# guzba/zippy

Measured on NVIDIA H100. Metric: compress_level1_gzip_input_throughput, higher is better.
Workload: dtype u8

## Files before the change

zippy_b200/csrc/zb_deflate.cu:

```cuda
#include "zb_device.cuh"
#include "zb_kernels.h"

#define LZ_THREADS (ZB_WARPS_PER_CHUNK * 32)
#define LZ_HASH_BITS 11
#define LZ_TABLE_ENTRIES (1 << LZ_HASH_BITS)
#define LZ_PRESEED 2048
#ifndef ZB_LZ1_RESOLVE_WINNER
#define ZB_LZ1_RESOLVE_WINNER 0
#endif
#define LZ_LANE_CAP 32

#define LZ_PIECE_BYTES ZB_REC_PIECE_BYTES
#define LZ_PHASES (ZB_SUB_BYTES / LZ_PIECE_BYTES)
#define LZ_PHASE_BYTES (ZB_CHUNK_BYTES / LZ_PHASES)
#define LZ_PHASE_HIST 1024
#define LZ_BATCH_LPW 2
#define LZ_BATCH_WINDOWS (32 / LZ_BATCH_LPW)
static_assert(LZ_PIECE_BYTES * ZB_WARPS_PER_CHUNK == LZ_PHASE_BYTES, "one piece per warp and phase");
static_assert(LZ_PIECE_BYTES / ZB_WINDOW % LZ_BATCH_WINDOWS == 0, "a batch of windows never straddles two pieces");

#define LZ_SM_DATA 0
#define LZ_SM_DATA_BYTES (LZ_PHASE_BYTES + LZ_PHASE_HIST + 64 + 384)
#define LZ_SM_TABLE (LZ_SM_DATA + LZ_SM_DATA_BYTES)
#define LZ_SM_TABLE_BYTES (ZB_WARPS_PER_CHUNK * LZ_TABLE_ENTRIES * 2)
#define LZ_SM_HIST (LZ_SM_TABLE + LZ_SM_TABLE_BYTES)
#define LZ_SM_HIST_BYTES (ZB_WARPS_PER_CHUNK * ZB_HIST_WORDS * 4)
#define LZ_SM_RING (LZ_SM_HIST + LZ_SM_HIST_BYTES)
#define LZ_SM_RING_BYTES (ZB_WARPS_PER_CHUNK * LZ_BATCH_WINDOWS * ZB_MATCH_SLOTS * 4)
#define LZ_SM_LMUL (LZ_SM_RING + LZ_SM_RING_BYTES)
#define LZ_LMUL_PIECE 33
#define LZ_LMUL_PQ 49
#define LZ_SM_LMUL_BYTES (56 * 4)
#define LZ_SM_PART (LZ_SM_LMUL + LZ_SM_LMUL_BYTES)
#define LZ_SM_PART_BYTES (ZB_WARPS_PER_CHUNK * 24)
#define LZ_SM_BAR (LZ_SM_PART + LZ_SM_PART_BYTES)
#define LZ_SM_TOTAL (LZ_SM_BAR + 16)
static_assert(LZ_TABLE_ENTRIES * 2 >= 4096, "a warp's table region must hold the CRC step table");
static_assert(3 * (LZ_SM_TOTAL + 1024) <= 233472, "three CTAs per SM");
static_assert(LZ_SM_PART % 8 == 0 && LZ_SM_TABLE % 16 == 0, "alignment");

__device__ __forceinline__ uint32_t lz_hash(uint32_t v) { return (v * 0x9E3779B1u) >> (32 - LZ_HASH_BITS); }
__device__ __forceinline__ uint32_t shl_clamp(uint32_t x, uint32_t n) {
  uint32_t r;
  asm("shl.b32 %0, %1, %2;" : "=r"(r) : "r"(x), "r"(n));
  return r;
}
__device__ __forceinline__ uint32_t low_mask(uint32_t n) { return shl_clamp(1u, n) - 1u; }

__device__ __forceinline__ uint32_t lz_final_rec(uint32_t mlen, uint32_t dist, int &lc, int &dc) {
  uint32_t le, de;
  lc = (int)zb_len_code_bf(mlen, le);
  dc = (int)zb_dist_code_bf(dist, de);
  return (uint32_t)lc | (le << 5) | ((uint32_t)dc << 10) | (de << 15);
}


__device__ __forceinline__ void lz_select(const uint8_t *data, uint32_t off0, uint32_t wb, uint32_t b1, uint32_t cur,
                                          uint32_t nvalid, uint32_t &m, uint32_t dist, uint32_t *ring_slot,
                                          uint32_t &sel, uint32_t &ism, uint32_t &endw) {
  const int lane = zb_lane();
  const uint32_t mm = __ballot_sync(ZB_FULL, m != 0);
  endw = 0;
  ism = 0;
  if (mm) {
    const uint32_t lbit = 1u << lane;
    const uint32_t endp = (uint32_t)lane + m;
    const uint32_t rest = shl_clamp(1u, endp) ? (mm >> endp) : 0u;
    uint32_t nc = rest ? endp + (uint32_t)(__ffs((int)rest) - 1) : 32u;
    uint32_t vis = 1u << (cur + (uint32_t)(__ffs((int)(mm >> cur)) - 1));
#pragma unroll
    for (int r = 0; r < 3; r++) {
      vis |= __reduce_or_sync(ZB_FULL, (vis & lbit) ? shl_clamp(1u, nc) : 0u);
      const uint32_t t = __shfl_sync(ZB_FULL, nc, (int)(nc & 31u));
      nc = nc < 32u ? t : 32u;
    }
    ism = vis;
    const int lastm = 31 - __clz((int)ism);
    const uint32_t cov = (ism & lbit) ? (low_mask(endp) & ~low_mask((uint32_t)lane)) : 0u;
    const uint32_t covered = __reduce_or_sync(ZB_FULL, cov);
    uint32_t mlast = __shfl_sync(ZB_FULL, m, lastm);
    if (mlast >= LZ_LANE_CAP) {
      const uint32_t md = __shfl_sync(ZB_FULL, dist, lastm);
      const uint32_t pos = wb + (uint32_t)lastm;
      const uint32_t off = off0 + pos + LZ_LANE_CAP + 8u * (uint32_t)lane;
      uint32_t x0 = zb_ld32_unaligned(data, off) ^ zb_ld32_unaligned(data, off - md);
      uint32_t x1 = zb_ld32_unaligned(data, off + 4) ^ zb_ld32_unaligned(data, off + 4 - md);
      uint32_t nm = x0 ? ((uint32_t)(__ffs((int)x0) - 1) >> 3) : 4u + (x1 ? ((uint32_t)(__ffs((int)x1) - 1) >> 3) : 4u);
      uint32_t stop = __ballot_sync(ZB_FULL, nm < 8u);
      if (stop) {
        int first = __ffs((int)stop) - 1;
        mlast = LZ_LANE_CAP + 8u * (uint32_t)first + __shfl_sync(ZB_FULL, nm, first);
      } else {
        mlast = LZ_LANE_CAP + 256u;
      }
      mlast = min(mlast, min((uint32_t)ZB_MAX_MATCH, b1 - pos));
      if (lane == lastm) m = mlast;
    }
    sel = ism | (~covered & ~low_mask(cur) & low_mask(nvalid));
    endw = (uint32_t)lastm + mlast;
    if (ism & lbit) {
      uint32_t rank = (uint32_t)__popc(ism & (lbit - 1u));
      ring_slot[rank] = (m - 3u) | ((dist - 1u) << 9);
    }
  } else {
    sel = low_mask(nvalid) & ~low_mask(cur);
  }
}

template <int LPW, bool LITS>
__device__ __forceinline__ void lz_batch_pass(const uint8_t *wdata, bool active, uint32_t ksel, uint32_t kism,
                                              const uint32_t *ring_win, uint32_t *whist, uint2 *gmask_w,
                                              uint32_t *grecs_piece, uint32_t &rec_base) {
  constexpr int NW = 32 / LPW;
  const uint32_t part = (uint32_t)zb_lane() / NW, wi = (uint32_t)zb_lane() % NW;
  if (active && part == 0) *gmask_w = make_uint2(ksel, kism);
  const uint32_t im = active ? kism : 0u;
  const uint32_t pm = (0xffffffffu >> (32 - 32 / LPW)) << (part * (32 / LPW));
  uint32_t s = (LITS && active) ? (ksel & ~kism & pm) : 0u;
  while (s) {
    const uint32_t bit = (uint32_t)(__ffs((int)s) - 1);
    s &= s - 1;
    const uint32_t sy = wdata[bit];
    atomicAdd(&whist[sy >> 1], 1u << ((sy & 1u) * 16u));
  }
  const uint32_t nmatch = (uint32_t)__popc(im);
  uint32_t incl = nmatch;
#pragma unroll
  for (int o = 1; o < NW; o <<= 1) {
    const uint32_t t = __shfl_up_sync(ZB_FULL, incl, o, NW);
    if (wi >= (uint32_t)o) incl += t;
  }
  uint32_t *grecs_w = grecs_piece + rec_base + incl - nmatch;
  rec_base += __shfl_sync(ZB_FULL, incl, NW - 1);
  for (uint32_t k = part; k < nmatch; k += LPW) {
    const uint32_t raw = ring_win[k];
    int lc, dc;
    const uint32_t fin = lz_final_rec((raw & 511u) + 3u, (raw >> 9) + 1u, lc, dc);
    grecs_w[k] = fin;
    const uint32_t s1 = 257u + (uint32_t)lc, s2 = (uint32_t)ZB_NUM_LITLEN + (uint32_t)dc;
    atomicAdd(&whist[s1 >> 1], 1u << ((s1 & 1u) * 16u));
    atomicAdd(&whist[s2 >> 1], 1u << ((s2 & 1u) * 16u));
  }
}

#ifndef ZB_LZ1_STAGE_CLOCKS
#define ZB_LZ1_STAGE_CLOCKS 0
#endif
enum { LZS_WAIT, LZS_CHECKSUM, LZS_SEED, LZS_PROBE, LZS_EXTEND, LZS_SELECT, LZS_BATCH, LZS_BARRIER, LZS_N };
#if ZB_LZ1_STAGE_CLOCKS
__device__ unsigned long long zb_lz1_stage_clk[LZS_N];
#define LZ_CLK_DECL                          \
  unsigned long long clk_acc[LZS_N] = {};    \
  long long clk_t = clock64();
#define LZ_CLK(s)                            \
// ... 397 lines not shown
    lz2_clear_table(own);
    __syncthreads();
    if (rlen) {
      zb_mbar_wait(bar, phase);
      phase ^= 1u;
    }

    const uint32_t b0 = (uint32_t)warp * ZB_SUB_BYTES;
    const uint32_t b1 = min(b0 + ZB_SUB_BYTES, len);
    {
      ZbCheck c;
      c.crc_raw = 0;
      c.a_sum = c.b_sum = 0;
      uint32_t n = b0 < len ? b1 - b0 : 0;
      if (n) {
        c = zb_warp_checksums(data, off0 + b0, n, crc_tab, lane_mul);
        const uint32_t after = len - b1;
        if (after) {
          const uint32_t shift = ((after & (ZB_SUB_BYTES - 1)) == 0) ? lane_mul[33 + after / ZB_SUB_BYTES] : zb_xpow8_t(tabs->pow2, after);
          c.crc_raw = zb_gf2_mul(c.crc_raw, shift);
          c.b_sum += (uint64_t)after * c.a_sum;
        }
      }
      if (lane == 0) {
        part[warp * 3 + 0] = c.crc_raw;
        part[warp * 3 + 1] = c.a_sum;
        part[warp * 3 + 2] = c.b_sum;
      }
      __syncwarp();
    }

    {
      const uint32_t nseg = (hg + rlen + LZ2_SEG_BYTES - 1) / LZ2_SEG_BYTES;
      for (uint32_t sg = (uint32_t)warp; sg + 1 < nseg; sg += ZB_WARPS_PER_CHUNK) {
        uint2 *tab = stat + (size_t)sg * LZ2_BUCKETS;
        lz2_clear_table(tab, (1 << LZ2_STATIC_BITS) * 2);
        __syncwarp();
        uint16_t *tab16 = reinterpret_cast<uint16_t *>(tab);
        const uint32_t q0 = sg ? sg * LZ2_SEG_BYTES - hg : 0u, q1 = (sg + 1) * LZ2_SEG_BYTES - hg;
        for (uint32_t s = q0; s < q1; s += 32) {
          const uint32_t q = s + (uint32_t)lane;
          const uint32_t v = zb_ld32_unaligned(data, mis + q);
          const uint32_t hs = lz2_hash_mul(v) >> (32 - LZ2_STATIC_BITS);
          const bool can = q + 4 <= rlen && q < q1;
          const uint32_t grp = __match_any_sync(ZB_FULL, can ? hs : (0x80000000u | (uint32_t)lane));
          if (can && lane == 31 - __clz((int)grp)) __stcg(&tab16[hs], (uint16_t)q);
        }
        __syncwarp();
      }
    }
    __syncthreads();

    if (b0 < len) {
      const uint32_t myseg = (hg + hb + b0) / LZ2_SEG_BYTES;
      uint32_t entry = b0;
      uint32_t ksel = 0, kism = 0;
      uint2 *gmask = masks + (size_t)chunk * ZB_WINDOWS_PER_CHUNK;
      uint32_t *grecs = recs + (size_t)chunk * ZB_RECS_PER_CHUNK;
      uint32_t rec_base = 0;
      for (uint32_t wb = b0; wb < b1; wb += 32) {
        const uint32_t win = wb >> 5, slot = win & (LZ2_RING_WINDOWS - 1u);
        if ((wb & (ZB_REC_PIECE_BYTES - 1u)) == 0u) rec_base = 0;
        const uint32_t p = wb + (uint32_t)lane;
        const uint32_t q = hb + p;
        const uint32_t v = zb_ld32_unaligned(data, off0 + p);
        const bool can = (p + 4 <= len);
        const uint32_t h = lz2_hash(v);
        const uint32_t limit = p < b1 ? min((uint32_t)ZB_MAX_MATCH, b1 - p) : 0u;
        const bool search = entry < wb + 32 && can && p >= entry && limit >= ZB_MIN_MATCH;
        const uint32_t hs = lz2_hash_mul(v) >> (32 - LZ2_STATIC_BITS);
        uint32_t hcand[4];
#pragma unroll
        for (int j = 0; j < 4; j++) {
          hcand[j] = 0xffffu;
          if (search && myseg > (uint32_t)j && prm.hist_segs > (uint32_t)j)
            hcand[j] = __ldcg(reinterpret_cast<const uint16_t *>(stat + (size_t)(myseg - 1u - (uint32_t)j) * LZ2_BUCKETS) + hs);
        }
        uint32_t grp;
        const uint2 bucket = lz2_probe_insert(own, h, can, q - (uint32_t)lane, grp);
        uint32_t sel = 0, ism = 0;
        if (entry < wb + 32) {
          const uint32_t nvalid = min(32u, b1 - wb);
          const uint32_t cur = entry - wb;
          uint32_t m = 0, dist = 1;
          int budget = search ? (int)prm.maxcand : 0;
          Lz2Pos P;
          P.data32 = reinterpret_cast<const uint32_t *>(data);
          P.poff = off0 + p;
          P.q = q;
          P.v = v;
          P.lim = min(q, (uint32_t)ZB_MAX_DIST);
          P.limit = limit;
          P.stop = min(limit, (uint32_t)LZ_LANE_CAP);
          uint32_t nl = 0;
          {
            const uint32_t lower = grp & ((1u << lane) - 1u);
            lz2_verify(P, q - ((uint32_t)lane - (uint32_t)(31 - __clz((int)(lower | 1u)))), search && lower != 0u, dlist, nl);
            lz2_verify(P, bucket.x & 0xffffu, search, dlist, nl);
            if (prm.own_ways > 1) lz2_verify(P, bucket.x >> 16, search, dlist, nl);
            if (prm.own_ways > 2) lz2_verify(P, bucket.y & 0xffffu, search, dlist, nl);
            if (prm.own_ways > 3) lz2_verify(P, bucket.y >> 16, search, dlist, nl);
#pragma unroll
            for (int j = 0; j < 4; j++)
              if (prm.hist_segs > (uint32_t)j) lz2_verify(P, hcand[j], search, dlist, nl);
          }
          const uint32_t rounds = __reduce_max_sync(ZB_FULL, nl);
          for (uint32_t k = 0; k < rounds; k++) {
            if (k < nl && budget > 0 && m < P.stop) lz2_extend(P, data, dlist[k * (uint32_t)LZ_THREADS], prm.good, m, dist, budget);
          }
          const uint32_t mnext = __shfl_down_sync(ZB_FULL, m, 1);
          if (lane < 31 && m != 0 && m < prm.lazy && mnext > m) m = 0;
          uint32_t endw;
          lz_select(data, off0, wb, b1, cur, nvalid, m, dist, ring + slot * ZB_MATCH_SLOTS, sel, ism, endw);
          entry = wb + max(endw, nvalid);
        }
        const uint32_t bl = (uint32_t)lane & (LZ2_RING_WINDOWS - 1u);
        if (bl == slot) {
          ksel = sel;
          kism = ism;
        }
        if (slot == LZ2_RING_WINDOWS - 1u || wb + 32 >= b1) {
          __syncwarp();
          const uint32_t bwin = win - slot + bl;
          lz_batch_pass<32 / LZ2_RING_WINDOWS, true>(data + off0 + (bwin << 5), bl <= slot, ksel, kism, ring + bl * ZB_MATCH_SLOTS,
                                               whist, gmask + bwin,
                                               grecs + ((wb & ~(uint32_t)(ZB_REC_PIECE_BYTES - 1u)) >> 2), rec_base);
          ksel = kism = 0;
          __syncwarp();
        }
      }
    }
    __syncthreads();
    {
      uint32_t *gh = reinterpret_cast<uint32_t *>(hist + (size_t)chunk * ZB_WARPS_PER_CHUNK * ZB_HIST_SYMS);
      for (int i = tid; i < ZB_WARPS_PER_CHUNK * ZB_HIST_WORDS; i += LZ_THREADS) gh[i] = hist_all[i];
    }
    if (tid == 0) {
      uint32_t raw = 0;
      uint64_t a = 0, b = 0;
      for (int w = 0; w < ZB_WARPS_PER_CHUNK; w++) {
        raw ^= (uint32_t)part[w * 3 + 0];
        a += part[w * 3 + 1];
        b += part[w * 3 + 2];
      }
      ZbChunkCheck cc;
      cc.crc_raw = raw;
      cc.adler = zb_adler_from_sums(a % ZB_ADLER_MOD, b % ZB_ADLER_MOD, len);
      chk[chunk] = cc;
    }
    __syncthreads();
  }
}

__global__ void __launch_bounds__(64)
    k_huff(const ZbChunkDesc *__restrict__ desc, const uint16_t *__restrict__ hist, ZbCodebook *__restrict__ cb,
           uint32_t n_chunks, int level) {
  uint32_t c = blockIdx.x * blockDim.x + threadIdx.x;
  if (c >= n_chunks) return;
  ZbChunkDesc d = desc[c];
  zb_build_codebook(hist + (size_t)c * ZB_WARPS_PER_CHUNK * ZB_HIST_SYMS, d.len, (d.flags & ZB_CHUNK_LAST) ? 1 : 0,
                    level == 0 ? 0 : -1, &cb[c]);
}

__device__ __forceinline__ uint32_t frame_head_bytes(int fmt, const uint8_t *fname_len, uint32_t m) {
  if (fmt == ZB_DF_GZIP) return 10u + (fname_len ? (uint32_t)fname_len[m] : 0u) + 1u;
  if (fmt == ZB_DF_ZLIB) return 2u;
  return 0u;
}
__device__ __forceinline__ uint32_t frame_tail_bytes(int fmt) {
  return fmt == ZB_DF_GZIP ? 8u : fmt == ZB_DF_ZLIB ? 4u : 0u;
}

#define SCAN_THREADS 1024
__global__ void __launch_bounds__(SCAN_THREADS)
    k_scan(ZbCompressWork w) {
  __shared__ uint64_t warp_tot[32];
  __shared__ uint64_t carry_s;
  const int tid = (int)threadIdx.x, lane = tid & 31, warp = tid >> 5;
  if (tid == 0) carry_s = w.out_base_ptr ? *w.out_base_ptr : w.out_base;
  __syncthreads();
  for (uint32_t base = 0; base < w.n_chunks; base += SCAN_THREADS) {
    uint32_t c = base + (uint32_t)tid;
    uint64_t sz = 0;
    uint32_t head = 0, flags = 0, member = 0;
    if (c < w.n_chunks) {
      ZbChunkDesc d = w.desc[c];
      flags = d.flags;
      member = d.member;
      sz = w.cb[c].total_bytes;
      if (flags & ZB_CHUNK_HEAD) {
        head = frame_head_bytes(w.data_format, w.fname_len, member);
        sz += head;
      }
      if (flags & ZB_CHUNK_LAST) sz += frame_tail_bytes(w.data_format);
    }
    uint64_t incl = sz;
#pragma unroll
    for (int o = 1; o < 32; o <<= 1) {
      uint64_t t = __shfl_up_sync(ZB_FULL, incl, o);
      if (lane >= o) incl += t;
    }
    if (lane == 31) warp_tot[warp] = incl;
    __syncthreads();
    if (warp == 0) {
      uint64_t t = warp_tot[lane], it = t;
#pragma unroll
      for (int o = 1; o < 32; o <<= 1) {
        uint64_t u = __shfl_up_sync(ZB_FULL, it, o);
        if (lane >= o) it += u;
      }
      warp_tot[lane] = it - t;
    }
    __syncthreads();
    uint64_t carry = carry_s;
    uint64_t excl = carry + warp_tot[warp] + incl - sz;
    if (c < w.n_chunks) {
      w.chunk_off[c] = excl + head;
      if (flags & ZB_CHUNK_FIRST) w.member_off[member] = excl;
    }
    __syncthreads();
    if (tid == SCAN_THREADS - 1) carry_s = excl + sz;
    __syncthreads();
  }
  if (tid == 0) w.member_off[w.n_members] = carry_s;
}

__global__ void __launch_bounds__(128)
    k_member_check(ZbCompressWork w) {
  const uint32_t m = (blockIdx.x * blockDim.x + threadIdx.x) >> 5, lane = threadIdx.x & 31u;
  if (m >= w.n_members) return;
  const uint32_t c0 = w.member_first[m], c1 = w.member_first[m + 1];
  const uint32_t per = (c1 - c0 + 31u) / 32u;
  const uint32_t a = min(c1, c0 + lane * per), b = min(c1, a + per);
  uint32_t raw = 0, ad = 1;
  uint64_t bytes = 0;
  for (uint32_t c = a; c < b; c++) {
    const uint32_t l = w.desc[c].len;
    const ZbChunkCheck cc = w.chk[c];
    if (w.data_format == ZB_DF_ZLIB) ad = zb_adler32_combine(ad, cc.adler, l);
    else if (w.data_format == ZB_DF_GZIP)
      raw = zb_gf2_mul(raw, l == ZB_CHUNK_BYTES ? w.tabs->sub_mul[0] : zb_xpow8_t(w.tabs->pow2, l)) ^ cc.crc_raw;
    bytes += l;
  }
  if (c1 - c0 > 1u) {
    for (int o = 1; o < 32; o <<= 1) {
      const uint32_t r_raw = __shfl_down_sync(0xffffffffu, raw, o), r_ad = __shfl_down_sync(0xffffffffu, ad, o);
      const uint64_t r_bytes = __shfl_down_sync(0xffffffffu, bytes, o);
      if ((lane & (uint32_t)(2 * o - 1)) == 0u && r_bytes) {
        if (w.data_format == ZB_DF_ZLIB) ad = zb_adler32_combine(ad, r_ad, r_bytes);
        else if (w.data_format == ZB_DF_GZIP) raw = zb_gf2_mul(raw, zb_xpow8_t(w.tabs->pow2, r_bytes)) ^ r_raw;
        bytes += r_bytes;
      }
    }
  }
  if (lane == 0) {
    if (w.carry_in) {
      const ZbMemberCarry ci = w.carry_in[m];
      if (w.data_format == ZB_DF_ZLIB) ad = zb_adler32_combine(ci.adler, ad, bytes);
      else if (w.data_format == ZB_DF_GZIP) raw = zb_gf2_mul(ci.crc_raw, zb_xpow8_t(w.tabs->pow2, bytes)) ^ raw;
      bytes += ci.bytes;
    }
    if (w.carry_out) {
      ZbMemberCarry co;
      co.crc_raw = raw;
      co.adler = ad;
      co.bytes = bytes;
      w.carry_out[m] = co;
    }
    uint32_t v = 0;
    if (w.data_format == ZB_DF_ZLIB) v = ad;
    else if (w.data_format == ZB_DF_GZIP)
      v = ~(zb_gf2_mul(bytes == ZB_CHUNK_BYTES ? w.tabs->sub_mul[0] : zb_xpow8_t(w.tabs->pow2, bytes), 0xffffffffu) ^ raw);
    w.member_check[m] = v;
    w.member_isize[m] = (uint32_t)bytes;
  }
}

#define PK_ROW_WORDS 17
#define PK_STG_WORDS (PK_ROW_WORDS * 32 + 4)
#define PK_EDGES 10
#define PK_LIT_OFF 1
#define PK_SLOT_WORDS 9
#define PK_REC_OFF (PK_LIT_OFF + 32 * PK_SLOT_WORDS)
static_assert(PK_REC_OFF + 32 * ZB_MATCH_SLOTS + 1 <= PK_STG_WORDS, "a batch's staged inputs fit in stg");
#define PK_CODE_NONE 320

struct PkEdges {
  uint32_t word[PK_EDGES];
  uint32_t val[PK_EDGES];
  uint32_t used[PK_EDGES];
};
__device__ __forceinline__ void pk_edge_or(PkEdges *ed, uint32_t relword, uint32_t bits) {
  int k = 0;
#pragma unroll
  for (int i = PK_EDGES - 1; i >= 0; i--)
    if (ed->word[i] == relword) k = i;
  atomicOr(&ed->val[k], bits);
  ed->used[k] = 1u;
}

__device__ __forceinline__ void pk_append(uint32_t *stg, const uint32_t *rows, uint32_t mybits, uint32_t &bitcur,
                                          uint32_t &sw0, uint32_t piece_start, uint32_t *dstw_rel, PkEdges *ed) {
  const int lane = zb_lane();
  uint32_t incl = mybits;
#pragma unroll
  for (int o = 1; o < 32; o <<= 1) {
    const uint32_t t = __shfl_up_sync(ZB_FULL, incl, o);
    if (lane >= o) incl += t;
  }
  const uint32_t total = __shfl_sync(ZB_FULL, incl, 31);
  uint32_t pos = bitcur + incl - mybits - sw0 * 32u;
  for (uint32_t k = 0; k * 32u < mybits; k++) {
    const uint32_t nb = min(32u, mybits - k * 32u);
    uint32_t v = rows[k * 32 + lane];
    if (nb < 32u) v &= (1u << nb) - 1u;
// ... 138 lines not shown
      uint32_t rec_base = 0;
      for (uint32_t wbase = 0; wbase < nwin; wbase += 32) {
        if (wbase && (wbase & (ZB_REC_PIECE_WINDOWS - 1u)) == 0u) {
          grecs += ZB_REC_PIECE_BYTES / 4;
          rec_base = 0;
        }
        const uint32_t widx = wbase + (uint32_t)lane;
        const uint32_t win = (b0 >> 5) + widx;
        uint2 mk = make_uint2(0u, 0u);
        if (widx < nwin) mk = gmask[win];
        uint32_t s = mk.x;
        const uint32_t im = mk.y;
        const uint32_t nmatch = (uint32_t)__popc(im);
        uint32_t rincl = nmatch;
#pragma unroll
        for (int o = 1; o < 32; o <<= 1) {
          const uint32_t t = __shfl_up_sync(ZB_FULL, rincl, o);
          if (lane >= o) rincl += t;
        }
        const uint32_t rtot = __shfl_sync(ZB_FULL, rincl, 31);
        {
          const uint32_t bbase = b0 + (wbase << 5);
          const uint32_t *pw = reinterpret_cast<const uint32_t *>(src + bbase - mis);
          const uint32_t nword = min(1024u, b1 - bbase) + mis;
#pragma unroll 1
          for (uint32_t k = (uint32_t)lane; 4u * k < nword; k += 32) {
            const uint32_t v = __ldg(pw + k);
            uint32_t *q = stg + PK_LIT_OFF + k + (k >> 3);
            if (k < 256u) *q = v;
            if (k && (k & 7u) == 0u) q[-1] = v;
          }
          const uint32_t *brec = grecs + rec_base;
#pragma unroll 1
          for (uint32_t k = (uint32_t)lane; k < rtot; k += 32) stg[PK_REC_OFF + k] = brec[k];
        }
        rec_base += rtot;
        __syncwarp();
        const uint8_t *lit = reinterpret_cast<const uint8_t *>(stg + PK_LIT_OFF + lane * PK_SLOT_WORDS) + mis;
        uint32_t ri = PK_REC_OFF + rincl - nmatch;
        uint32_t wi = (uint32_t)lane, acc = 0, accn = 0;
        while (s) {
          const uint32_t t1 = s & (0u - s);
          s ^= t1;
          const uint32_t t2 = s & (0u - s);
          const uint32_t l1 = lit[31 - __clz(t1)], l2 = lit[31 - __clz(t2)];
          const uint32_t r = stg[ri];
          const bool is_m = (im & t1) != 0u;
          const bool pair = t2 != 0u && (im & (t1 | t2)) == 0u;
          s ^= pair ? t2 : 0u;
          ri += is_m ? 1u : 0u;
          const uint32_t rec = is_m ? r : 0u;
          const uint32_t sym1 = is_m ? 257u + (rec & 31u) : l1;
          const uint32_t sym2 = is_m ? 288u + ((rec >> 10) & 31u) : pair ? l2 : PK_CODE_NONE;
          const uint32_t e1 = codes[sym1], e2 = codes[sym2];
          pk_put(rows, (e1 & 0xffffu) | ((rec >> 5) & 31u) << __byte_perm(e1, 0u, 0x4442), e1 >> 24, acc, accn, wi);
          pk_put(rows, (e2 & 0xffffu) | (rec >> 15) << __byte_perm(e2, 0u, 0x4442), e2 >> 24, acc, accn, wi);
        }
        rows[wi] = acc;
        __syncwarp();
        for (uint32_t k = (uint32_t)lane; k < PK_REC_OFF - PK_LIT_OFF + rtot; k += 32) stg[PK_LIT_OFF + k] = 0u;
        __syncwarp();
        pk_append(stg, rows, wi - (uint32_t)lane + accn, bitcur, sw0, piece_start, dstw_rel, &ed);
      }
    }
    if (lane == 0 && (bitcur & 31u)) pk_edge_or(&ed, sw0, stg[0]);
  }
  if (tid == 96) {
    const uint32_t e = codes[256];
    uint32_t pos = B0 + cb->eob_bit_start;
    unsigned long long tv = (unsigned long long)(e & 0xffffu);
    uint32_t nb = e >> 24;
    if (!cb->is_final) {
      nb += 3u;
      nb += (8u - ((pos + nb) & 7u)) & 7u;
      tv |= 0xffff0000ull << nb;
      nb += 32u;
    } else {
      nb += (8u - ((pos + nb) & 7u)) & 7u;
    }
    while (nb) {
      const uint32_t rel = pos >> 5, sh = pos & 31u, take = min(nb, 32u - sh);
      const uint32_t bits = (uint32_t)(tv & ((1ull << take) - 1ull)) << sh;
      if (sh == 0 && take == 32u) dstw_rel[rel] = bits;
      else pk_edge_or(&ed, rel, bits);
      tv >>= take;
      pos += take;
      nb -= take;
    }
  }
  __syncthreads();
  if (tid < PK_EDGES && ed.used[tid] && (tid == 0 || ed.word[tid] != ed.word[tid - 1])) {
    const uint32_t rel = ed.word[tid], val = ed.val[tid];
    const uint32_t lo = rel * 32u, hi = lo + 32u;
    if (lo >= B0 && hi <= end_bit) dstw_rel[rel] = val;
    else {
      uint8_t *bp = reinterpret_cast<uint8_t *>(dstw_rel + rel);
      for (uint32_t j = 0; j < 4; j++)
        if (lo + 8u * j >= B0 && lo + 8u * j + 8u <= end_bit) bp[j] = (uint8_t)(val >> (8u * j));
    }
  }
}

static bool zb_is_lz_level(int level) { return level == -1 || level >= 2; }
ZbLz2Params zb_lz2_params(int level) {
  static const ZbLz2Params table[10] = {{4, 4, 4, 8, 16}, {4, 4, 4, 8, 16}, {2, 4, 2, 4, 0},  {2, 4, 3, 4, 6},   {3, 4, 3, 4, 8},
                                        {3, 4, 4, 8, 16}, {4, 4, 4, 8, 16}, {4, 4, 6, 8, 32}, {4, 4, 8, 16, 32}, {4, 4, 8, 32, 64}};
  return table[(level >= 2 && level <= 9) ? level : 6];
}
size_t zb_lz2_table_bytes(int *grid_out) {
  int grid = LZ2_CTAS_PER_SM * zb_sm_count();
  if (grid_out) *grid_out = grid;
  return (size_t)grid * LZ2_TABLES_PER_CTA * LZ2_BUCKETS * sizeof(uint2);
}
typedef void (*ZbLzKernel)(const uint8_t *, const ZbChunkDesc *, uint2 *, uint32_t *, uint16_t *, ZbChunkCheck *,
                           const ZbCrcTables *);
static ZbLzKernel zb_lz_kernel(int mode, int data_format) {
  const int ck = data_format == ZB_DF_GZIP ? ZB_CK_CRC : data_format == ZB_DF_ZLIB ? ZB_CK_ADLER : 0;
  if (mode) return ck == ZB_CK_CRC ? k_lz<1, ZB_CK_CRC> : ck == ZB_CK_ADLER ? k_lz<1, ZB_CK_ADLER> : k_lz<1, 0>;
  return ck == ZB_CK_CRC ? k_lz<0, ZB_CK_CRC> : ck == ZB_CK_ADLER ? k_lz<0, ZB_CK_ADLER> : k_lz<0, 0>;
}
cudaError_t zb_setup_deflate_attrs() {
  cudaError_t e = cudaSuccess;
  static const int fmts[3] = {ZB_DF_GZIP, ZB_DF_ZLIB, ZB_DF_DEFLATE};
  for (int mode = 0; mode < 2; mode++)
    for (int f = 0; f < 3; f++) {
      const ZbLzKernel k = zb_lz_kernel(mode, fmts[f]);
      if (e == cudaSuccess) e = cudaFuncSetAttribute(k, cudaFuncAttributeMaxDynamicSharedMemorySize, LZ_SM_TOTAL);
      if (e == cudaSuccess) e = cudaFuncSetAttribute(k, cudaFuncAttributePreferredSharedMemoryCarveout, cudaSharedmemCarveoutMaxShared);
    }
  if (e == cudaSuccess) e = cudaFuncSetAttribute(k_lz2, cudaFuncAttributeMaxDynamicSharedMemorySize, LZ2_SM_TOTAL);
  cudaFuncAttributes fa;
  if (e == cudaSuccess) e = cudaFuncGetAttributes(&fa, k_huff);
  if (e == cudaSuccess) e = cudaFuncGetAttributes(&fa, k_scan);
  if (e == cudaSuccess) e = cudaFuncGetAttributes(&fa, k_member_check);
  if (e == cudaSuccess) e = cudaFuncGetAttributes(&fa, k_pack);
  return e;
}
cudaError_t zb_launch_lz(const ZbCompressWork &w, cudaStream_t s) {
  if (w.n_chunks == 0) return cudaSuccess;
  if (zb_is_lz_level(w.level)) {
    int grid = 0;
    (void)zb_lz2_table_bytes(&grid);
    if ((uint32_t)grid > w.n_chunks) grid = (int)w.n_chunks;
    k_lz2<<<grid, LZ_THREADS, LZ2_SM_TOTAL, s>>>(w.src, w.desc, w.masks, w.recs, w.hist, w.chk, w.tabs, w.lz2_tables,
                                                 w.n_chunks, zb_lz2_params(w.level));
  } else {
    const ZbLzKernel k = zb_lz_kernel((w.level == -2 || w.level == 0) ? 0 : 1, w.data_format);
    k<<<w.n_chunks, LZ_THREADS, LZ_SM_TOTAL, s>>>(w.src, w.desc, w.masks, w.recs, w.hist, w.chk, w.tabs);
  }
  return cudaGetLastError();
}
cudaError_t zb_launch_huff(const ZbCompressWork &w, cudaStream_t s) {
  if (w.n_chunks == 0) return cudaSuccess;
  k_huff<<<(w.n_chunks + 63) / 64, 64, 0, s>>>(w.desc, w.hist, w.cb, w.n_chunks, w.level);
  return cudaGetLastError();
}
cudaError_t zb_launch_scan(const ZbCompressWork &w, cudaStream_t s) {
  k_scan<<<1, SCAN_THREADS, 0, s>>>(w);
  if (w.n_members) k_member_check<<<(w.n_members + 3) / 4, 128, 0, s>>>(w);
  return cudaGetLastError();
}
cudaError_t zb_launch_pack(const ZbCompressWork &w, cudaStream_t s) {
  if (w.n_chunks == 0) return cudaSuccess;
  k_pack<<<w.n_chunks, LZ_THREADS, 0, s>>>(w);
  return cudaGetLastError();
}
```

Measured before the change: 74.42.

## Build Huffman codebooks with one warp per chunk instead of one thread

Replaces the per-thread codebook builder with a warp-cooperative version. Histogram summing, the rank-based sort, length assignment, canonical code generation, header bit packing and per-warp bit offsets are all spread across lanes and use shared memory per warp. This targets the serial per-thread Huffman construction, which left the huff kernel with few active threads and long latency. The tree build and RLE stay on a single lane, and the added shared-memory footprint and warp synchronisation cost something in return. Optional stage clock instrumentation is compiled out by default.

After: 77.09 (median of 6 runs). +3.6%, better.

```diff
diff --git a/zippy_b200/csrc/zb_deflate.cu b/zippy_b200/csrc/zb_deflate.cu
--- a/zippy_b200/csrc/zb_deflate.cu
+++ b/zippy_b200/csrc/zb_deflate.cu
@@ -1,5 +1,6 @@
 #include "zb_device.cuh"
 #include "zb_kernels.h"
+#include "zb_huff_warp.cuh"
 
 #define LZ_THREADS (ZB_WARPS_PER_CHUNK * 32)
 #define LZ_HASH_BITS 11
@@ -703,15 +704,13 @@
   }
 }
 
-__global__ void __launch_bounds__(64)
-    k_huff(const ZbChunkDesc *__restrict__ desc, const uint16_t *__restrict__ hist, ZbCodebook *__restrict__ cb,
-           uint32_t n_chunks, int level) {
-  uint32_t c = blockIdx.x * blockDim.x + threadIdx.x;
-  if (c >= n_chunks) return;
-  ZbChunkDesc d = desc[c];
-  zb_build_codebook(hist + (size_t)c * ZB_WARPS_PER_CHUNK * ZB_HIST_SYMS, d.len, (d.flags & ZB_CHUNK_LAST) ? 1 : 0,
-                    level == 0 ? 0 : -1, &cb[c]);
-}
+#if ZB_HUFF_STAGE_CLOCKS
+extern "C" int zb200_huff_stage_clocks(unsigned long long *out) {
+  unsigned long long zero[HWS_N] = {};
+  if (cudaMemcpyFromSymbol(out, zb_huff_stage_clk, sizeof(zero)) != cudaSuccess) return -1;
+  return cudaMemcpyToSymbol(zb_huff_stage_clk, zero, sizeof(zero)) == cudaSuccess ? 0 : -1;
+}
+#endif
 
 __device__ __forceinline__ uint32_t frame_head_bytes(int fmt, const uint8_t *fname_len, uint32_t m) {
   if (fmt == ZB_DF_GZIP) return 10u + (fname_len ? (uint32_t)fname_len[m] : 0u) + 1u;
@@ -1156,7 +1155,7 @@
 }
 cudaError_t zb_launch_huff(const ZbCompressWork &w, cudaStream_t s) {
   if (w.n_chunks == 0) return cudaSuccess;
-  k_huff<<<(w.n_chunks + 63) / 64, 64, 0, s>>>(w.desc, w.hist, w.cb, w.n_chunks, w.level);
+  k_huff<<<(w.n_chunks + HW_WARPS - 1) / HW_WARPS, HW_WARPS * 32, 0, s>>>(w.desc, w.hist, w.cb, w.n_chunks, w.level);
   return cudaGetLastError();
 }
 cudaError_t zb_launch_scan(const ZbCompressWork &w, cudaStream_t s) {
diff --git a/zippy_b200/csrc/zb_huff_warp.cuh b/zippy_b200/csrc/zb_huff_warp.cuh
--- /dev/null
+++ b/zippy_b200/csrc/zb_huff_warp.cuh
@@ -0,0 +1,510 @@
+#pragma once
+#include <stddef.h>
+
+#include "zb_device.cuh"
+#include "zb_kernels.h"
+
+#define HW_WARPS 4
+
+static_assert(offsetof(ZbCodebook, dd) == 288 * 4 && offsetof(ZbCodebook, block_type) == 320 * 4 &&
+                  offsetof(ZbCodebook, warp_bit_start) == 322 * 4 && offsetof(ZbCodebook, chunk_len) == 333 * 4 &&
+                  offsetof(ZbCodebook, hdr) == 334 * 4 && sizeof(ZbCodebook) == 418 * 4,
+              "k_huff stores the codebook as 418 words: ll, dd, 14 scalars, 84 header words");
+#define HW_TAIL_WORDS (418 - 320)
+
+struct __align__(16) HwWarp {
+  uint32_t key[320];
+  uint32_t skey[320];
+  uint32_t a[320];
+  uint8_t lens[320];
+  uint32_t num_ll[36], num_d[36];
+  uint32_t clf[20];
+};
+#define HW_K_RSYM 0
+#define HW_K_REXT 80
+#define HW_K_CKEY 160
+#define HW_K_CSKEY 184
+#define HW_K_CA 208
+#define HW_K_NUMC 232
+#define HW_K_CLL 268
+#define HW_K_CLC 276
+static_assert(HW_K_CLC + 20 <= 320, "code-length arrays fit in key[]");
+#define HW_S_TAIL 0
+#define HW_S_CNT 100
+#define HW_S_NXT 116
+
+#ifndef ZB_HUFF_STAGE_CLOCKS
+#define ZB_HUFF_STAGE_CLOCKS 0
+#endif
+enum { HWS_SUM, HWS_SORT, HWS_MK, HWS_LIMIT, HWS_ASSIGN, HWS_RLE, HWS_CL, HWS_HEADER, HWS_CODES, HWS_BITS, HWS_STORE, HWS_N };
+#if ZB_HUFF_STAGE_CLOCKS
+__device__ unsigned long long zb_huff_stage_clk[HWS_N];
+#endif
+struct HwClk {
+#if ZB_HUFF_STAGE_CLOCKS
+  unsigned long long acc[HWS_N];
+  long long t;
+  __device__ __forceinline__ void start() {
+#pragma unroll
+    for (int s = 0; s < HWS_N; s++) acc[s] = 0;
+    t = clock64();
+  }
+  __device__ __forceinline__ void mark(int s) {
+    const long long n = clock64();
+    acc[s] += (unsigned long long)(n - t);
+    t = n;
+  }
+  __device__ __forceinline__ void publish() {
+    if (zb_lane() == 0)
+#pragma unroll
+      for (int s = 0; s < HWS_N; s++) atomicAdd(&zb_huff_stage_clk[s], acc[s]);
+  }
+#else
+  __device__ __forceinline__ void start() {}
+  __device__ __forceinline__ void mark(int) {}
+  __device__ __forceinline__ void publish() {}
+#endif
+};
+
+__device__ __forceinline__ void hw_mk(uint32_t *a, int m, uint32_t *num) {
+  for (int i = 0; i <= 32; i++) num[i] = 0;
+  if (m < 2) return;
+  if (m == 2) {
+    num[1] = 2;
+    return;
+  }
+  a[0] += a[1];
+  int root = 0, leaf = 2;
+  for (int next = 1; next < m - 1; next++) {
+    if (leaf >= m || a[root] < a[leaf]) {
+      a[next] = a[root];
+      a[root++] = (uint32_t)next;
+    } else {
+      a[next] = a[leaf++];
+    }
+    if (leaf >= m || (root < next && a[root] < a[leaf])) {
+      a[next] += a[root];
+      a[root++] = (uint32_t)next;
+    } else {
+      a[next] += a[leaf++];
+    }
+  }
+  a[m - 2] = 0;
+  for (int next = m - 3; next >= 0; next--) a[next] = a[a[next]] + 1;
+  int avbl = 1, used = 0, dpth = 0, root2 = m - 2;
+  while (avbl > 0) {
+    while (root2 >= 0 && (int)a[root2] == dpth) {
+      used++;
+      root2--;
+    }
+    if (avbl > used) num[dpth > 32 ? 32 : dpth] += (uint32_t)(avbl - used);
+    avbl = 2 * used;
+    dpth++;
+    used = 0;
+  }
+}
+
+__device__ __forceinline__ void hw_limit(uint32_t *num, int m, int limit) {
+  if (m < 2) return;
+  for (int l = limit + 1; l <= 32; l++) {
+    num[limit] += num[l];
+    num[l] = 0;
+  }
+  uint32_t total = 0;
+  for (int l = limit; l >= 1; l--) total += num[l] << (limit - l);
+  while (total > (1u << limit)) {
+    num[limit]--;
+    for (int l = limit - 1; l >= 1; l--)
+      if (num[l]) {
+        num[l]--;
+        num[l + 1] += 2;
+        break;
+      }
+    total--;
+  }
+}
+
+__device__ __forceinline__ uint32_t hw_len_at(const uint32_t *num, int limit, uint32_t j) {
+  uint32_t l = (uint32_t)limit, c = num[limit];
+  while (j >= c) c += num[--l];
+  return l;
+}
+
+__device__ __forceinline__ void hw_or_bits(uint32_t *w, uint32_t bit, uint32_t v, uint32_t n) {
+  const uint32_t sh = bit & 31u;
+  atomicOr(&w[bit >> 5], v << sh);
+  if (sh + n > 32u) atomicOr(&w[(bit >> 5) + 1], v >> (32u - sh));
+}
+
+__device__ __forceinline__ void hw_canon(const uint8_t *lens, int n, uint32_t *out, uint32_t *cnt, uint32_t *nxt) {
+  const int lane = zb_lane();
+  const uint32_t lt = (1u << lane) - 1u;
+  if (lane < 16) cnt[lane] = 0;
+  __syncwarp();
+  for (int base = 0; base < n; base += 32) {
+    const int s = base + lane;
+    const uint32_t l = s < n ? lens[s] : 0u;
+    const uint32_t peers = __match_any_sync(ZB_FULL, l);
+    if (l && lane == 31 - __clz((int)peers)) cnt[l] += (uint32_t)__popc(peers);
+    __syncwarp();
+  }
+  if (lane >= 1 && lane < 16) {
+    uint32_t nx = 0;
+    for (int k = 1; k < lane; k++) nx = (nx + cnt[k]) << 1;
+    nxt[lane] = nx;
+  }
+  __syncwarp();
+  for (int base = 0; base < n; base += 32) {
+    const int s = base + lane;
+    const uint32_t l = s < n ? lens[s] : 0u;
+    const uint32_t peers = __match_any_sync(ZB_FULL, l);
+    const uint32_t code = l ? nxt[l] + (uint32_t)__popc(peers & lt) : 0u;
+    __syncwarp();
+    if (l && lane == 31 - __clz((int)peers)) nxt[l] += (uint32_t)__popc(peers);
+    __syncwarp();
+    if (s < n) out[s] = l ? (zb_brev16(code, (int)l) | (l << 16)) : 0u;
+  }
+}
+
+__device__ __forceinline__ uint32_t hw_cost(const uint8_t *lens, int s) {
+  return s < ZB_NUM_LITLEN ? lens[s] + (s > 256 ? (uint32_t)zb_len_extra_bits(s - 257) : 0u)
+                           : lens[288 + s - ZB_NUM_LITLEN] + (uint32_t)zb_dist_extra_bits(s - ZB_NUM_LITLEN);
+}
+
+__device__ __forceinline__ void hw_build_codebook(HwWarp &ws, const uint32_t *__restrict__ hw, uint32_t chunk_len,
+                                                  uint32_t is_final, int force_type, ZbCodebook *cb, HwClk &clk) {
+  const int lane = zb_lane();
+  const uint32_t lt = (1u << lane) - 1u;
+  uint32_t *gw = reinterpret_cast<uint32_t *>(cb);
+  const uint32_t npieces = chunk_len == 0 ? 1u : (chunk_len + 65534u) / 65535u;
+  const uint64_t stored_bytes = (uint64_t)chunk_len + 5ull * npieces;
+  if (force_type == 0) {
+    for (int i = lane; i < 418; i += 32)
+      gw[i] = i == 331 ? (uint32_t)stored_bytes : i == 332 ? is_final : i == 333 ? chunk_len : 0u;
+    return;
+  }
+
+  uint32_t fa[5], fb[5];
+#pragma unroll
+  for (int k = 0; k < 5; k++) {
+    const int p = lane + 32 * k;
+    uint32_t lo = 0, hi = 0;
+    if (p < ZB_HIST_WORDS)
+#pragma unroll
+      for (int w = 0; w < ZB_WARPS_PER_CHUNK; w++) {
+        const uint32_t v = __ldg(hw + w * ZB_HIST_WORDS + p);
+        lo += v & 0xffffu;
+        hi += v >> 16;
+      }
+    fa[k] = p == 128 ? 1u : lo;
+    fb[k] = hi;
+  }
+  {
+    uint32_t *l32 = reinterpret_cast<uint32_t *>(ws.lens);
+    for (int i = lane; i < 80; i += 32) l32[i] = 0;
+  }
+  clk.mark(HWS_SUM);
+
+  int m = 0, mll = 0;
+#pragma unroll
+  for (int k = 0; k < 5; k++) {
+    const uint32_t s0 = 2u * (uint32_t)(lane + 32 * k);
+    const bool u0 = fa[k] != 0, u1 = fb[k] != 0;
+    const uint32_t b0 = __ballot_sync(ZB_FULL, u0), b1 = __ballot_sync(ZB_FULL, u1);
+    const int at = m + __popc(b0 & lt) + __popc(b1 & lt);
+    const bool isd = s0 >= ZB_NUM_LITLEN;
+    const uint32_t kb = (isd ? 0x80000000u : 0u) | (isd ? s0 - ZB_NUM_LITLEN : s0);
+    if (u0) ws.key[at] = kb | (fa[k] << 9);
+    if (u1) ws.key[at + (u0 ? 1 : 0)] = (kb + 1u) | (fb[k] << 9);
+    m += __popc(b0) + __popc(b1);
+    const uint32_t llm = k < 4 ? ZB_FULL : 0x7fffu;
+    mll += __popc(b0 & llm) + __popc(b1 & llm);
+  }
+  if (lane < 4) ws.key[m + lane] = 0xffffffffu;
+  __syncwarp();
+  {
+    const uint4 *q4 = reinterpret_cast<const uint4 *>(ws.key);
+    const int nq = (m + 3) >> 2;
+    for (int base = 0; base < m; base += 64) {
+      const int i0 = base + lane, i1 = i0 + 32;
+      const uint32_t k0 = i0 < m ? ws.key[i0] : 0u, k1 = i1 < m ? ws.key[i1] : 0u;
+      uint32_t r0 = 0, r1 = 0;
+      for (int j = 0; j < nq; j++) {
+        const uint4 q = q4[j];
+        r0 += (uint32_t)(q.x < k0) + (uint32_t)(q.y < k0) + (uint32_t)(q.z < k0) + (uint32_t)(q.w < k0);
+        r1 += (uint32_t)(q.x < k1) + (uint32_t)(q.y < k1) + (uint32_t)(q.z < k1) + (uint32_t)(q.w < k1);
+      }
+      if (i0 < m) ws.skey[r0] = k0;
+      if (i1 < m) ws.skey[r1] = k1;
+    }
+  }
+  __syncwarp();
+  for (int i = lane; i < m; i += 32) ws.a[i] = (ws.skey[i] >> 9) & 0x3fffffu;
+  __syncwarp();
+  clk.mark(HWS_SORT);
+
+  const int md = m - mll;
+  if (lane < 2) hw_mk(lane ? ws.a + mll : ws.a, lane ? md : mll, lane ? ws.num_d : ws.num_ll);
+  __syncwarp();
+  clk.mark(HWS_MK);
+  if (lane < 2) hw_limit(lane ? ws.num_d : ws.num_ll, lane ? md : mll, 15);
+  __syncwarp();
+  clk.mark(HWS_LIMIT);
+
+  uint32_t dyn_payload, fix_payload, extra;
+  {
+    uint32_t dyn = 0, fix = 0, ext = 0;
+    for (int i = lane; i < m; i += 32) {
+      const uint32_t k = ws.skey[i];
+      const bool isd = i >= mll;
+      const int mx = isd ? md : mll;
+      const uint32_t l = mx >= 2 ? hw_len_at(isd ? ws.num_d : ws.num_ll, 15, (uint32_t)(isd ? i - mll : i)) : 1u;
+      const uint32_t f = (k >> 9) & 0x3fffffu, s = k & 511u;
+      ws.lens[isd ? 288 + s : s] = (uint8_t)l;
+      dyn += f * l;
+      fix += f * (isd ? 5u : (uint32_t)zb_fixed_ll_len((int)s));
+      ext += f * (uint32_t)(isd ? zb_dist_extra_bits((int)s) : s > 256 ? zb_len_extra_bits((int)s - 257) : 0);
+    }
+    if (lane == 0) {
+      if (mll < 2) {
+        const uint32_t s = mll ? ws.skey[0] & 511u : 0u;
+        ws.lens[s == 0 ? 1 : 0] = 1;
+        if (!mll) ws.lens[0] = 1;
+      }
+      if (md < 2) {
+        const uint32_t s = md ? ws.skey[mll] & 511u : 0u;
+        ws.lens[288 + (s == 0 ? 1 : 0)] = 1;
+        if (!md) ws.lens[288] = 1;
+      }
+    }
+    dyn_payload = __reduce_add_sync(ZB_FULL, dyn);
+    fix_payload = __reduce_add_sync(ZB_FULL, fix);
+    extra = __reduce_add_sync(ZB_FULL, ext);
+  }
+  if (lane < 19) ws.clf[lane] = 0;
+  __syncwarp();
+  int nll, nd;
+  {
+    uint32_t hi = 0;
+    for (int s = lane; s < ZB_NUM_LITLEN; s += 32)
+      if (ws.lens[s]) hi = (uint32_t)s + 1u;
+    nll = max(257, (int)__reduce_max_sync(ZB_FULL, hi));
+    nd = max(1, (int)__reduce_max_sync(ZB_FULL, (lane < ZB_NUM_DIST && ws.lens[288 + lane]) ? (uint32_t)lane + 1u : 0u));
+  }
+  clk.mark(HWS_ASSIGN);
+
+  uint8_t *rsym = reinterpret_cast<uint8_t *>(ws.key + HW_K_RSYM);
+  uint8_t *rext = reinterpret_cast<uint8_t *>(ws.key + HW_K_REXT);
+  int nr = 0;
+  if (lane == 0) {
+    const int nseq = nll + nd;
+    auto seq = [&](int i) { return (int)ws.lens[i < nll ? i : 288 + i - nll]; };
+    auto emit = [&](int sy, int ex) {
+      rsym[nr] = (uint8_t)sy;
+      rext[nr++] = (uint8_t)ex;
+      ws.clf[sy]++;
+    };
+    for (int i = 0; i < nseq;) {
+      const int v = seq(i);
+      int run = 1;
+      while (i + run < nseq && seq(i + run) == v) run++;
+      int left = run;
+      if (v == 0) {
+        while (left >= 11) {
+          const int r = left > 138 ? 138 : left;
+          emit(18, r - 11);
+          left -= r;
+        }
+        if (left >= 3) {
+          emit(17, left - 3);
+          left = 0;
+        }
+        while (left-- > 0) emit(0, 0);
+      } else {
+        emit(v, 0);
+        left--;
+        while (left >= 3) {
+          const int r = left > 6 ? 6 : left;
+          emit(16, r - 3);
+          left -= r;
+        }
+        while (left-- > 0) emit(v, 0);
+      }
+      i += run;
+    }
+  }
+  nr = __shfl_sync(ZB_FULL, nr, 0);
+  __syncwarp();
+  clk.mark(HWS_RLE);
+
+  uint32_t *ckey = ws.key + HW_K_CKEY, *cskey = ws.key + HW_K_CSKEY, *ca = ws.key + HW_K_CA, *num_c = ws.key + HW_K_NUMC;
+  uint8_t *cll = reinterpret_cast<uint8_t *>(ws.key + HW_K_CLL);
+  uint32_t *clc = ws.key + HW_K_CLC;
+  uint32_t *cnt = ws.skey + HW_S_CNT, *nxt = ws.skey + HW_S_NXT;
+  {
+    const uint32_t cf = lane < 19 ? ws.clf[lane] : 0u;
+    const uint32_t bm = __ballot_sync(ZB_FULL, cf != 0);
+    const int mc = __popc(bm);
+    if (cf) ckey[__popc(bm & lt)] = (cf << 9) | (uint32_t)lane;
+    if (lane < 4) ckey[mc + lane] = 0xffffffffu;
+    if (lane < 5) reinterpret_cast<uint32_t *>(cll)[lane] = 0;
+    __syncwarp();
+    if (lane < mc) {
+      const uint32_t k = ckey[lane];
+      const uint4 *q4 = reinterpret_cast<const uint4 *>(ckey);
+      uint32_t r = 0;
+      for (int j = 0; j < (mc + 3) >> 2; j++) {
+        const uint4 q = q4[j];
+        r += (uint32_t)(q.x < k) + (uint32_t)(q.y < k) + (uint32_t)(q.z < k) + (uint32_t)(q.w < k);
+      }
+      cskey[r] = k;
+      ca[r] = k >> 9;
+    }
+    __syncwarp();
+    if (lane == 0) {
+      hw_mk(ca, mc, num_c);
+      hw_limit(num_c, mc, 7);
+    }
+    __syncwarp();
+    if (lane < mc) cll[cskey[lane] & 511u] = (uint8_t)(mc >= 2 ? hw_len_at(num_c, 7, (uint32_t)lane) : 1u);
+    if (lane == 0 && mc < 2) {
+      const uint32_t s = mc ? cskey[0] & 511u : 0u;
+      cll[s == 0 ? 1 : 0] = 1;
+      if (!mc) cll[0] = 1;
+    }
+    __syncwarp();
+    hw_canon(cll, 19, clc, cnt, nxt);
+    __syncwarp();
+  }
+  clk.mark(HWS_CL);
+
+  const int jo = lane - 3;
+  const int ord = lane < 3 ? 16 + lane : jo == 0 ? 0 : (jo & 1) ? 8 + (jo >> 1) : 8 - (jo >> 1);
+  const uint32_t ordlen = lane < 19 ? cll[ord] : 0u;
+  const int hclen = max(4, (int)__reduce_max_sync(ZB_FULL, ordlen ? (uint32_t)lane + 1u : 0u));
+  uint32_t dyn_hdr;
+  {
+    uint32_t wsum = 0;
+    for (int i = lane; i < nr; i += 32) {
+      const int sy = rsym[i];
+      wsum += cll[sy] + (sy == 16 ? 2u : sy == 17 ? 3u : sy == 18 ? 7u : 0u);
+    }
+    dyn_hdr = 17u + 3u * (uint32_t)hclen + __reduce_add_sync(ZB_FULL, wsum);
+  }
+  const uint64_t dyn_bits = dyn_hdr + (uint64_t)dyn_payload + extra;
+  const uint64_t fix_bits = 3 + (uint64_t)fix_payload + extra;
+  const uint64_t dyn_bytes = is_final ? (dyn_bits + 7) / 8 : (dyn_bits + 3 + 7) / 8 + 4;
+  const uint64_t fix_bytes = is_final ? (fix_bits + 7) / 8 : (fix_bits + 3 + 7) / 8 + 4;
+  int type = 2;
+  uint64_t best = dyn_bytes;
+  if (fix_bytes < best) {
+    type = 1;
+    best = fix_bytes;
+  }
+  if (stored_bytes <= best) {
+    type = 0;
+    best = stored_bytes;
+  }
+  uint32_t *tail = ws.skey + HW_S_TAIL, *hdr = tail + 14;
+  for (int i = lane; i < HW_TAIL_WORDS - 14; i += 32) hdr[i] = 0;
+  __syncwarp();
+  uint32_t hdr_bits = 0;
+  if (type == 1) {
+    if (lane == 0) hdr[0] = is_final | 2u;
+    hdr_bits = 3;
+    for (int s = lane; s < 320; s += 32) ws.lens[s] = (uint8_t)(s < 288 ? zb_fixed_ll_len(s) : 5);
+  } else if (type == 2) {
+    if (lane == 0)
+      hdr[0] = is_final | 4u | (uint32_t)(nll - 257) << 3 | (uint32_t)(nd - 1) << 8 | (uint32_t)(hclen - 4) << 13;
+    __syncwarp();
+    if (lane < hclen) hw_or_bits(hdr, 17u + 3u * (uint32_t)lane, ordlen, 3);
+    uint32_t pos = 17u + 3u * (uint32_t)hclen;
+    for (int base = 0; base < nr; base += 32) {
+      const int i = base + lane;
+      uint32_t w = 0, v = 0;
+      if (i < nr) {
+        const int sy = rsym[i];
+        const uint32_t cl = cll[sy];
+        w = cl + (sy == 16 ? 2u : sy == 17 ? 3u : sy == 18 ? 7u : 0u);
+        v = (clc[sy] & 0xffffu) | (uint32_t)rext[i] << cl;
+      }
+      uint32_t incl = w;
+#pragma unroll
+      for (int o = 1; o < 32; o <<= 1) {
+        const uint32_t t = __shfl_up_sync(ZB_FULL, incl, o);
+        if (lane >= o) incl += t;
+      }
+      if (w) hw_or_bits(hdr, pos + incl - w, v, w);
+      pos += __shfl_sync(ZB_FULL, incl, 31);
+    }
+    hdr_bits = pos;
+  }
+  __syncwarp();
+  clk.mark(HWS_HEADER);
+
+  if (type == 0) {
+    for (int i = lane; i < 320; i += 32) gw[i] = 0;
+  } else {
+    hw_canon(ws.lens, 288, gw, cnt, nxt);
+    hw_canon(ws.lens + 288, 32, gw + 288, cnt, nxt);
+  }
+  clk.mark(HWS_CODES);
+
+  uint32_t wbs[ZB_WARPS_PER_CHUNK], eob = 0;
+#pragma unroll
+  for (int w = 0; w < ZB_WARPS_PER_CHUNK; w++) wbs[w] = 0;
+  if (type != 0) {
+    uint32_t part[ZB_WARPS_PER_CHUNK];
+#pragma unroll
+    for (int w = 0; w < ZB_WARPS_PER_CHUNK; w++) part[w] = 0;
+#pragma unroll
+    for (int k = 0; k < 5; k++) {
+      const int p = lane + 32 * k;
+      if (p < ZB_HIST_WORDS) {
+        const uint32_t c0 = hw_cost(ws.lens, 2 * p), c1 = hw_cost(ws.lens, 2 * p + 1);
+#pragma unroll
+        for (int w = 0; w < ZB_WARPS_PER_CHUNK; w++) {
+          const uint32_t v = __ldg(hw + w * ZB_HIST_WORDS + p);
+          part[w] += (v & 0xffffu) * c0 + (v >> 16) * c1;
+        }
+      }
+    }
+    uint32_t pos = hdr_bits;
+#pragma unroll
+    for (int w = 0; w < ZB_WARPS_PER_CHUNK; w++) {
+      wbs[w] = pos;
+      pos += __reduce_add_sync(ZB_FULL, part[w]);
+    }
+    eob = pos;
+  }
+  clk.mark(HWS_BITS);
+
+  if (lane == 0) {
+    tail[0] = (uint32_t)type;
+    tail[1] = hdr_bits;
+#pragma unroll
+    for (int w = 0; w < ZB_WARPS_PER_CHUNK; w++) tail[2 + w] = wbs[w];
+    tail[10] = eob;
+    tail[11] = (uint32_t)best;
+    tail[12] = is_final;
+    tail[13] = chunk_len;
+  }
+  __syncwarp();
+  for (int i = lane; i < HW_TAIL_WORDS; i += 32) gw[320 + i] = tail[i];
+  clk.mark(HWS_STORE);
+}
+
+__global__ void __launch_bounds__(HW_WARPS * 32)
+    k_huff(const ZbChunkDesc *__restrict__ desc, const uint16_t *__restrict__ hist, ZbCodebook *__restrict__ cb,
+           uint32_t n_chunks, int level) {
+  __shared__ HwWarp ws_all[HW_WARPS];
+  const uint32_t warp = threadIdx.x >> 5;
+  const uint32_t c = blockIdx.x * HW_WARPS + warp;
+  if (c >= n_chunks) return;
+  const ZbChunkDesc d = desc[c];
+  HwClk clk;
+  clk.start();
+  hw_build_codebook(ws_all[warp], reinterpret_cast<const uint32_t *>(hist) + (size_t)c * ZB_WARPS_PER_CHUNK * ZB_HIST_WORDS,
+                    d.len, (d.flags & ZB_CHUNK_LAST) ? 1u : 0u, level == 0 ? 0 : -1, &cb[c], clk);
+  clk.publish();
+}
```
